# addtt/ladder-vae-pytorch

Measured on AMD Instinct MI355X. Metric: training images/sec (ELBO step: fwd+bwd+Adamax), higher is better.
Workload: dtype f32; 1 GPU; CIFAR10-shaped 15-layer LVAE (BASELINE configs[2]): 32x32x3, zdims 32x15, 4 blocks/layer, 64 filters, gated+skip, DMoL-10, dropout 0.2, free bits 1.0; batch_per_gpu=256, global_batch=256, parallelism=dp1, hip_graph=True

## Files before the change

### ladder-vae-pytorch_amd/csrc/conv3x3_bf16.hip

```cpp
#include <string.h>

#include "bf16_frag.h"
#include "bn_stats.h"
#include "lvae_host.h"

namespace lvae {

struct BfArgs {
  lvae_conv_desc d;
  const __bf16* Wp;
  int TH, TW, NI, tiles_h, halo_w, halo_h, halo_px, ntn, flip, Cin;
  uint32_t m_thw, m_tw, m_per_img, m_halo_w, m_tiles_h;
  int bm;
  int debug;
};

constexpr int BF_LDK = 72;

template <int SPLIT, int MI, bool PRE = false, bool XB = false, bool YB = false>
__global__ __launch_bounds__(256, 2) void conv3x3_bf16_kernel(BfArgs a) {
  kernarg_warmup<(sizeof(BfArgs) < 1024 ? sizeof(BfArgs) : 1024)>();
  static_assert(SPLIT == 1 || (!XB && !YB), "bf16 storage exists for the bf16-operand form only");
  constexpr int BM = 64 * MI, LDK = BF_LDK;
  extern __shared__ __attribute__((aligned(16))) unsigned char smem_raw[];
// ... 701 lines not shown
#pragma unroll
    for (int r = 0; r < 16; ++r) acc[j][r] = 0.f;
  f32x4 bsum = zero4, bsum8 = zero4;

  auto stage = [&](BfHRegs<XB, DB>& R, __bf16* Xs) {
    if (dbg & 2) return;
    __bf16* Ds = Xs + a.halo_px * LDK;
#pragma unroll
    for (int u = 0; u < (XB ? 2 : 4); ++u) {
      const int px = xpx + (XB ? 128 : 64) * u;
      if (px < a.halo_px) {
        if (XB) {
          bf16x8 w = R.x8[XB ? u : 0];
          if (d.in_scale && !(dbg & 16)) {
            f32x4 lo = {(float)w[0], (float)w[1], (float)w[2], (float)w[3]}, hi = {(float)w[4], (float)w[5], (float)w[6], (float)w[7]};
            lo = act_fwd4(lo * sc0 + sh0, d.in_act);
            hi = act_fwd4(hi * sc1 + sh1, d.in_act);
            w = to_bf16x8(lo, hi);
          }
          if (!((R.xok >> u) & 1u)) w = zero8;
          *reinterpret_cast<bf16x8*>(Xs + px * LDK + xcl) = w;
        } else {
          f32x4 w = zero4;
          if ((R.xok >> u) & 1u) {
            w = R.x4[XB ? 0 : u];
            if (d.in_scale && !(dbg & 16)) w = act_fwd4(w * sc0 + sh0, d.in_act);
          }
          *reinterpret_cast<bf16x4*>(Xs + px * LDK + xcl) = to_bf16x4(w);
        }
      }
    }
#pragma unroll
    for (int u = 0; u < (DB ? 2 : 4); ++u) {
      const int p = dpx + (DB ? 64 : 32) * u;
      if (DB) {
        const bf16x8 w = ((R.dok >> u) & 1u) ? R.d8[DB ? u : 0] : zero8;
        bsum += f32x4{(float)w[0], (float)w[1], (float)w[2], (float)w[3]};
        bsum8 += f32x4{(float)w[4], (float)w[5], (float)w[6], (float)w[7]};
        *reinterpret_cast<bf16x8*>(Ds + p * LDK + dcl) = w;
      } else {
        const f32x4 w = ((R.dok >> u) & 1u) ? R.d4[DB ? 0 : u] : zero4;
        bsum += w;
        *reinterpret_cast<bf16x4*>(Ds + p * LDK + dcl) = to_bf16x4(w);
      }
    }
  };
  auto mma_tile = [&](const __bf16* Xs) {
    if (dbg & 1) return;
    const __bf16* Ds = Xs + a.halo_px * LDK;
    const __bf16* Dl = Ds + drow0 * LDK + chd;
    int tb[3];
#pragma unroll
    for (int j = 0; j < 3; ++j) {
      tb[j] = tapoff[j];
      asm volatile("" : "+s"(tb[j]));
    }
#pragma unroll
    for (int s = 0; s < KS; ++s) {
      const bf16x8 bfr = tr_frag(Dl + 16 * s * LDK, Dl + (16 * s + 4) * LDK);
#pragma unroll
      for (int j = 0; j < 3; ++j) {
        if (j < ntap) {
          const bf16x8 afr = tr_frag(Xs + xoff[s][0] + tb[j], Xs + xoff[s][1] + tb[j]);
          acc[j] = __builtin_amdgcn_mfma_f32_32x32x16_bf16(afr, bfr, acc[j], 0, 0, 0);
        }
      }
      if (s & 1) __builtin_amdgcn_sched_barrier(0);
    }
  };

  BfHRegs<XB, DB> R0, R1;
  const int stride = nrange;
  int tile = range;
  if (tile < a.ntiles) prefetch(tile, R0);
  if (tile + stride < a.ntiles) prefetch(tile + stride, R1);
  for (; tile < a.ntiles; tile += 2 * stride) {
    stage(R0, buf0);
    __syncthreads();
    if (tile + 2 * stride < a.ntiles) prefetch(tile + 2 * stride, R0);
    mma_tile(buf0);
    if (tile + stride >= a.ntiles) break;
    stage(R1, buf0 + img_elems);
    __syncthreads();
    if (tile + 3 * stride < a.ntiles) prefetch(tile + 3 * stride, R1);
    mma_tile(buf0 + img_elems);
  }

  float* sw = a.slab_w + (size_t)range * 9 * Cin * d.Cout;
#pragma unroll
  for (int j = 0; j < 3; ++j) {
    if (j < ntap) {
      const int tap = tap0 + j;
#pragma unroll
      for (int r = 0; r < 16; ++r) {
        const int ci = cih * 32 + (r & 3) + 8 * (r >> 2) + 4 * lh, co = coh * 32 + li;
        if (!(dbg & 8) || acc[j][r] == 12345.678f) sw[((size_t)tap * Cin + ci) * d.Cout + co] = acc[j][r];
      }
    }
  }
  if (a.slab_b && cih == 0) {
    __syncthreads();
    float* red = reinterpret_cast<float*>(smem_raw);
    constexpr int NG = DB ? 64 : 32;
    if (DB) {
      *reinterpret_cast<f32x4*>(red + dpx * 64 + dcl) = bsum;
      *reinterpret_cast<f32x4*>(red + dpx * 64 + dcl + 4) = bsum8;
    } else {
      *reinterpret_cast<f32x4*>(red + dpx * 64 + dcl) = bsum;
    }
    __syncthreads();
    if (t < 64) {
      float v = 0.f;
#pragma unroll
      for (int g = 0; g < NG; ++g) v += red[g * 64 + t];
      a.slab_b[(size_t)range * d.Cout + t] = v;
    }
  }
}


__device__ __forceinline__ void bf_prep_element(const BfPrepEntry& e, int idx) {
  const int k = idx & 63, n = idx >> 6;
  if (n >= e.Npad) return;
  const int ntn = e.Npad >> 6, tn = n >> 6, nn = n & 63;
  for (int tap = 0; tap < 9; ++tap) {
    float r = (n < e.N && k < e.K) ? e.w[tap * e.stap + (int64_t)k * e.sk + (int64_t)n * e.sn] : 0.f;
    __bf16* dst = e.U + ((size_t)((tap * ntn + tn) * 4 + (k >> 4)) * e.kind * 2 + (nn >> 5)) * 512 + (((k >> 3) & 1) * 32 + (nn & 31)) * 8 + (k & 7);
    for (int p = 0; p < e.kind; ++p) {
      const __bf16 b = (__bf16)r;
      dst[(size_t)p * 1024] = b;
      r -= (float)b;
    }
  }
}

__device__ __forceinline__ void gate_prep_element(const BfPrepEntry& e, int idx) {
  const int planes = e.kind & 31;
  const int k = idx % e.K, n = idx / e.K;
  if (n >= e.N) return;
  float r = e.w[(int64_t)k * e.sk + (int64_t)n * e.sn];
  __bf16* dst = e.U + ((size_t)((k >> 4) * (e.N >> 5) + (n >> 5)) * planes) * 512 + (((k >> 3) & 1) * 32 + (n & 31)) * 8 + (k & 7);
  for (int p = 0; p < planes; ++p) {
    const __bf16 b = (__bf16)r;
    dst[(size_t)p * 512] = b;
    r -= (float)b;
  }
}

__global__ __launch_bounds__(256) void bf_weight_kernel(BfPrepEntry e) {
  if (e.kind & 32) gate_prep_element(e, blockIdx.x * 256 + threadIdx.x);
  else bf_prep_element(e, blockIdx.x * 256 + threadIdx.x);
}

__global__ __launch_bounds__(256) void bf_weight_batched_kernel(const BfPrepEntry* __restrict__ entries) {
  const BfPrepEntry e = entries[blockIdx.y];
  if (e.kind == 33 || e.kind == 35) {
    gate_prep_element(e, blockIdx.x * 256 + threadIdx.x);
    return;
  }
  if (e.kind != 1 && e.kind != 3) return;
  bf_prep_element(e, blockIdx.x * 256 + threadIdx.x);
}

int conv3x3_bf16_prepare_batched(const void* entries, int n, int npad, hipStream_t s) {
  hipLaunchKernelGGL(bf_weight_batched_kernel, dim3((npad * 64 + 255) / 256, n), dim3(256), 0, s, static_cast<const BfPrepEntry*>(entries));
  LVAE_LAUNCH_CHECK("bf_weight_batched");
  return 0;
}

size_t conv3x3_bf16_workspace(const lvae_conv_desc* d, int split) {
  const int ntn = (d->Cout + 63) / 64;
  return (size_t)9 * ntn * split * 4096 * sizeof(__bf16);
}

void conv3x3_bf16_prep_entry(const lvae_conv_desc* d, int split, void* entry) {
  BfPrepEntry e;
  e.w = d->w;
  e.U = static_cast<__bf16*>(d->workspace);
  e.stap = d->w_stap;
  e.sk = d->w_sk;
  e.sn = d->w_sn;
  e.K = d->C1;
  e.N = d->Cout;
  e.Npad = (d->Cout + 63) / 64 * 64;
  e.flip = 0;
  e.Kpad = 64;
  e.kind = split;
  memcpy(entry, &e, sizeof(e));
}

size_t resblock_gate_ws_bytes(const lvae_conv_desc* d, int planes) { return (size_t)d->C1 * d->Cout * planes * sizeof(__bf16); }
void resblock_gate_prep_entry(const lvae_conv_desc* d, int planes, void* entry) {
  BfPrepEntry e;
  e.w = d->w;
  e.U = static_cast<__bf16*>(d->workspace);
  e.stap = 0;
  e.sk = d->w_sk;
  e.sn = d->w_sn;
  e.K = d->C1;
  e.N = d->Cout;
  e.Npad = d->Cout;
  e.flip = 0;
  e.Kpad = d->C1;
  e.kind = 32 + planes;
  memcpy(entry, &e, sizeof(e));
}
int resblock_gate_prepare_single(const lvae_conv_desc* d, int planes, hipStream_t s) {
  BfPrepEntry e;
  resblock_gate_prep_entry(d, planes, &e);
  hipLaunchKernelGGL(bf_weight_kernel, dim3((e.K * e.N + 255) / 256), dim3(256), 0, s, e);
  LVAE_LAUNCH_CHECK("gate_weight");
  return 0;
}

int conv3x3_bf16_prepare_single(const lvae_conv_desc* d, int split, hipStream_t s) {
  BfPrepEntry e;
  conv3x3_bf16_prep_entry(d, split, &e);
  hipLaunchKernelGGL(bf_weight_kernel, dim3((e.Npad * 64 + 255) / 256), dim3(256), 0, s, e);
  LVAE_LAUNCH_CHECK("bf_weight");
  return 0;
}

static size_t bf_lds_bytes(int split, int halo_px, int bm) {
  const size_t in = (size_t)split * halo_px * BF_LDK * 2;
  const size_t out = (size_t)bm * 68 * 4;
  return in > out ? in : out;
}

static bool bf_plan_bm(const lvae_conv_desc* d, int split, int BM, BfArgs& a) {
  const int N = d->N, H = d->H, W = d->W;
  if (W > BM) return false;
  int TH = 1;
  for (int c = 1; c <= H; ++c)
    if (H % c == 0 && c * W <= BM) TH = c;
  int NI = BM / (TH * W);
  if (NI < 1) NI = 1;
  if (TH < H) NI = 1;
  if (NI > N) NI = N;
  a.TH = TH;
  a.TW = W;
  a.NI = NI;
  a.tiles_h = H / TH;
  a.halo_h = TH + 2;
  a.halo_w = W + 2;
  a.halo_px = NI * a.halo_h * a.halo_w;
  a.m_thw = fastdiv_magic(TH * W);
  a.m_tw = fastdiv_magic(W);
  a.m_per_img = fastdiv_magic(a.halo_h * a.halo_w);
  a.m_halo_w = fastdiv_magic(a.halo_w);
  a.bm = BM;
  return bf_lds_bytes(split, a.halo_px, BM) <= 160 * 1024;
}

static bool bf_plan(const lvae_conv_desc* d, int split, BfArgs& a) {
  if (bf_plan_bm(d, split, 128, a) && bf_lds_bytes(split, a.halo_px, 128) <= 80 * 1024 &&
      (int64_t)((d->N + a.NI - 1) / a.NI) * a.tiles_h * ((d->Cout + 63) / 64) >= 256)
    return true;
  if (bf_plan_bm(d, split, 64, a)) return true;
  return bf_plan_bm(d, split, 128, a);
}

static bool bf_select(const lvae_conv_desc* d, int split, BfArgs& a) {
  const int Cin = d->C1;
  if (d->KH != 3 || d->KW != 3 || d->stride != 1 || d->pad != 1 || d->x2 != nullptr || d->OH != d->H || d->OW != d->W) return false;
  if (d->in_fold != nullptr) return false;
  if (Cin > 64 || Cin % 4 != 0 || d->Cout % 4 != 0) return false;
  if ((int64_t)d->N * d->H * d->W * Cin >= ((int64_t)1 << 31)) return false;
  if (!al16_or_null(d->x) || !al16_or_null(d->y) || !al16_or_null(d->bias) || !al16_or_null(d->out_scale) || !al16_or_null(d->in_scale) || !al16_or_null(d->in_shift) ||
      !al16_or_null(d->stats_pivot) || !al16_or_null(d->stats_x))
    return false;
  a.d = *d;
  a.Cin = Cin;
  a.flip = d->gather == LVAE_GATHER_TRANSPOSED ? 1 : 0;
  return bf_plan(d, split, a);
}

static bool conv3x3_bf16_eligible(const lvae_conv_desc* d, int split) {
  BfArgs a;
  return bf_select(d, split, a);
}

int conv3x3_bf16_form(const lvae_conv_desc* d) {
  if (d->precision == LVAE_PREC_BF16) return conv3x3_bf16_eligible(d, 1) ? 1 : 0;
  const bool split_on = d->form == LVAE_FORM_SIX_PRODUCT_DIRECT;
  static const int64_t min_m = tune("LVAE_F32_SPLIT_MIN_M", 256 * 64);
  if (!split_on || (int64_t)d->N * d->H * d->W < min_m) return 0;
  return conv3x3_bf16_eligible(d, 3) ? 3 : 0;
}

bool conv3x3_bf16_plan(const lvae_conv_desc* d, bool assume_ws, ConvPlan& p) {
  const int split = conv3x3_bf16_form(d);
  if (split == 0) return false;
  const size_t ws = conv3x3_bf16_workspace(d, split);
  if (!assume_ws && (d->workspace == nullptr || (size_t)d->workspace_bytes < ws || !al16_or_null(d->workspace))) return false;
  BfArgs a;
  bf_select(d, split, a);
  p = ConvPlan{};
  p.variant = split == 1 ? LVAE_VARIANT_BF16_DIRECT : LVAE_VARIANT_SIX_DIRECT;
  p.rows = ((d->N + a.NI - 1) / a.NI) * a.tiles_h;
  p.workspace = ws;
  return true;
}

template <int SPLIT, int MI, bool PRE = false, bool XB = false, bool YB = false>
static int launch_bf(BfArgs a, hipStream_t s) {
  const int img_groups = (a.d.N + a.NI - 1) / a.NI;
  a.ntn = (a.d.Cout + 63) / 64;
  a.d.in_fold = nullptr;
  return launch_lds<conv3x3_bf16_kernel<SPLIT, MI, PRE, XB, YB>>("conv3x3_bf16", dim3(img_groups * a.tiles_h * a.ntn), dim3(256), bf_lds_bytes(SPLIT, a.halo_px, 64 * MI), 160 * 1024, s, a);
}

int conv3x3_bf16_launch(const lvae_conv_desc* d, const ConvPlan& p, hipStream_t s) {
  const int split = p.variant == LVAE_VARIANT_BF16_DIRECT ? 1 : 3;
  BfArgs a;
  bf_select(d, split, a);
  if (!d->workspace_ready) {
    BfPrepEntry e;
    conv3x3_bf16_prep_entry(d, split, &e);
// ... 126 lines not shown
```

### ladder-vae-pytorch_amd/csrc/conv3x3_wino.hip

```cpp
#include <stdlib.h>
#include <string.h>

#include "bf16_frag.h"
#include "bn_stats.h"
#include "lvae_host.h"

#ifndef LVAE_W1_RING
#define LVAE_W1_RING 3
#endif

namespace lvae {

struct WinoArgs {
  lvae_conv_desc d;
  const float* U;
  int TH, TW, NI, tiles_h, halo_w, halo_h, halo_px, ntn, Npad, tiles_x, wt_per_img, n_wt, Cin;
  uint32_t m_thw, m_per_img, m_halo_w, m_tiles_x, m_wt_per_img, m_tw;
  lvae_bn_fold f;
  int store_pivot;
  const __bf16* g_ws;
  const float* g_bias;
  const float* g_res;
  float* g_ab;
  float* g_out;
  float* g_stats;
  const float* g_pivot;
  int g_act;
};

__device__ __forceinline__ void store_u_split(__bf16* U3, int NB, int p, int k, int n, float v) {
  const size_t base = (((size_t)(p * 4 + (k >> 4)) * NB + (n >> 5)) * 3 * 64 + ((k >> 3) & 1) * 32 + (n & 31)) * 8 + (k & 7);
  float r = v;
#pragma unroll
  for (int q = 0; q < 3; ++q) {
    const __bf16 b = (__bf16)r;
    U3[base + (size_t)q * 512] = b;
    r -= (float)b;
  }
}

__global__ __launch_bounds__(256) void wino_weight_kernel(const float* __restrict__ w, int64_t stap, int64_t sk, int64_t sn,
                                                           int K, int Kpad, int N, int Npad, int flip, float* __restrict__ U, int split) {
  const int idx = blockIdx.x * 256 + threadIdx.x;
  if (idx >= Npad * Kpad) return;
  const int e = idx & 3, n = (idx >> 2) % Npad, kq = (idx >> 2) / Npad;
  const int k = kq * 4 + e;
  float g[3][3];
#pragma unroll
  for (int a = 0; a < 3; ++a)
#pragma unroll
    for (int b = 0; b < 3; ++b) {
      const int tap = flip ? (2 - a) * 3 + (2 - b) : a * 3 + b;
      g[a][b] = (n < N && k < K) ? w[tap * stap + (int64_t)k * sk + (int64_t)n * sn] : 0.f;
    }
  float t[4][3];
#pragma unroll
  for (int b = 0; b < 3; ++b) {
    t[0][b] = g[0][b];
    t[1][b] = 0.5f * (g[0][b] + g[1][b] + g[2][b]);
    t[2][b] = 0.5f * (g[0][b] - g[1][b] + g[2][b]);
    t[3][b] = g[2][b];
  }
  const size_t slab = (size_t)Npad * Kpad;
#pragma unroll
  for (int a = 0; a < 4; ++a) {
    const float u0 = t[a][0], u1 = 0.5f * (t[a][0] + t[a][1] + t[a][2]), u2 = 0.5f * (t[a][0] - t[a][1] + t[a][2]), u3 = t[a][2];
    if (split) {
      __bf16* U3 = reinterpret_cast<__bf16*>(U);
      store_u_split(U3, Npad >> 5, a * 4, k, n, u0);
      store_u_split(U3, Npad >> 5, a * 4 + 1, k, n, u1);
      store_u_split(U3, Npad >> 5, a * 4 + 2, k, n, u2);
      store_u_split(U3, Npad >> 5, a * 4 + 3, k, n, u3);
    } else {
      float* dst = U + (size_t)(a * 4) * slab + idx;
      dst[0] = u0;
      dst[slab] = u1;
      dst[2 * slab] = u2;
      dst[3 * slab] = u3;
    }
  }
}

struct WinoPrepEntry {
  const float* w;
  float* U;
  int64_t stap, sk, sn;
  int32_t K, N, Npad, flip;
  int32_t Kpad, pad_;
};
static_assert(sizeof(WinoPrepEntry) == 64, "entry layout is part of the C ABI (lvae_conv2d_prepare_entry)");

__global__ __launch_bounds__(256) void wino_weight_batched_kernel(const WinoPrepEntry* __restrict__ entries) {
  const WinoPrepEntry e = entries[blockIdx.y];
  const int idx = blockIdx.x * 256 + threadIdx.x;
  if (e.pad_ != 0 && e.pad_ != 16) return;
  if (idx >= e.Npad * e.Kpad) return;
  const int c = idx & 3, n = (idx >> 2) % e.Npad, kq = (idx >> 2) / e.Npad;
  const int k = kq * 4 + c;
  float g[3][3];
#pragma unroll
  for (int a = 0; a < 3; ++a)
#pragma unroll
    for (int b = 0; b < 3; ++b) {
      const int tap = e.flip ? (2 - a) * 3 + (2 - b) : a * 3 + b;
      g[a][b] = (n < e.N && k < e.K) ? e.w[tap * e.stap + (int64_t)k * e.sk + (int64_t)n * e.sn] : 0.f;
    }
  float t[4][3];
#pragma unroll
  for (int b = 0; b < 3; ++b) {
    t[0][b] = g[0][b];
    t[1][b] = 0.5f * (g[0][b] + g[1][b] + g[2][b]);
    t[2][b] = 0.5f * (g[0][b] - g[1][b] + g[2][b]);
    t[3][b] = g[2][b];
  }
  const size_t slab = (size_t)e.Npad * e.Kpad;
#pragma unroll
  for (int a = 0; a < 4; ++a) {
    const float u0 = t[a][0], u1 = 0.5f * (t[a][0] + t[a][1] + t[a][2]), u2 = 0.5f * (t[a][0] - t[a][1] + t[a][2]), u3 = t[a][2];
    if (e.pad_ == 16) {
      __bf16* U3 = reinterpret_cast<__bf16*>(e.U);
      store_u_split(U3, e.Npad >> 5, a * 4, k, n, u0);
      store_u_split(U3, e.Npad >> 5, a * 4 + 1, k, n, u1);
      store_u_split(U3, e.Npad >> 5, a * 4 + 2, k, n, u2);
      store_u_split(U3, e.Npad >> 5, a * 4 + 3, k, n, u3);
    } else {
      float* dst = e.U + (size_t)(a * 4) * slab + idx;
      dst[0] = u0;
      dst[slab] = u1;
      dst[2 * slab] = u2;
      dst[3 * slab] = u3;
    }
  }
}

constexpr int WLDO = 68;

template <int NT>
__device__ __forceinline__ void wino_fold_bn(const lvae_bn_fold& f, int C, float* scratch, float* coef, int t, bool writer) {
  constexpr int G = NT / 32;
  const int q = t & 31, g = t >> 5, rows = f.rows;
  f32x4 s = {0.f, 0.f, 0.f, 0.f};
  if (2 * q < C)
    for (int r = g; r < rows; r += 8 * G) {
      f32x4 p[8];
#pragma unroll
      for (int u = 0; u < 8; ++u) {
        const int rr = r + u * G;
        p[u] = *reinterpret_cast<const f32x4*>(f.parts + ((size_t)(rr < rows ? rr : 0) * 2) * C + 4 * q);
      }
#pragma unroll
      for (int u = 0; u < 8; ++u)
        if (r + u * G < rows) s += p[u];
    }
  *reinterpret_cast<f32x4*>(scratch + g * 128 + 4 * q) = s;
  __syncthreads();
  if (t < C) {
    double sa = 0.0, sb = 0.0;
#pragma unroll
    for (int k = 0; k < G; ++k) {
      sa += (double)scratch[k * 128 + t];
      sb += (double)scratch[k * 128 + C + t];
    }
    const float pivot = f.parts[((size_t)rows * 2) * C + t];
    const float gam = f.gamma ? f.gamma[t] : 1.f, bet = f.beta ? f.beta[t] : 0.f;
    const BnChannel r = bn_finalize_channel(sa, sb, pivot, f.M, f.eps, gam, bet);
    coef[t] = r.scale;
    coef[64 + t] = r.shift;
    if (writer) {
      if (f.coef_out) bn_store_coef(f.coef_out, C, t, r);
      if (f.running_mean) bn_update_running(f.running_mean, f.running_var, t, f.running_mean[t], f.running_var[t], f.momentum, r, f.M);
    }
  }
  __syncthreads();
}

#if defined(LVAE_WINO_DBG) && (LVAE_WINO_DBG & 64)
__device__ unsigned long long g_wino_stamps[8192 * 8];
#define WINO_STAMP(i)                                                                                           \
  do {                                                                                                          \
    if ((threadIdx.x & 63) == 0 && blockIdx.x < 1024)                                                           \
      g_wino_stamps[(blockIdx.x * (blockDim.x >> 6) + (threadIdx.x >> 6)) * 8 + (i)] = __builtin_amdgcn_s_memtime(); \
  } while (0)
#else
#define WINO_STAMP(i) do {} while (0)
#endif

template <int CIN, int NH, int MT, bool SPL>
__global__ __launch_bounds__(256, MT == 1 ? 2 : 1) void conv3x3_wino_kernel(WinoArgs a) {
  kernarg_warmup<(sizeof(WinoArgs) < 1024 ? sizeof(WinoArgs) : 1024)>();
  static_assert(!SPL || (CIN == 64 && MT == 1 && NH == 2), "six-product form: 64 reduction channels, 128-pixel workgroups");
  constexpr int WLDA = CIN + 4;
  constexpr int KSTEPS = CIN / 8, NSLICE = CIN / 16;
  constexpr int CW = 32 * NH;
  constexpr int C4N = CW / 4;
  constexpr int PG = 256 / C4N;
  constexpr int NT = 32 * MT;
  constexpr int QN = 4 * NT / PG;
  constexpr int RING = NH == 1 ? 3 : 2;
  extern __shared__ __attribute__((aligned(16))) float smem[];
  float* As = smem;
  const lvae_conv_desc& d = a.d;
  const int t = threadIdx.x, lane = t & 63, wave = t >> 6;
  const int li = lane & 31, lh = lane >> 5;
#ifdef LVAE_WINO_DBG
  constexpr int dbg = LVAE_WINO_DBG;
#else
  constexpr int dbg = 0;
#endif
  WINO_STAMP(0);
  int bid = blockIdx.x;
  {
    const int nwg = gridDim.x, xcd = bid & 7, q = nwg >> 3, r = nwg & 7;
    bid = (xcd < r ? xcd * (q + 1) : r * (q + 1) + (xcd - r) * q) + (bid >> 3);
  }
  const int tile_n = bid % a.ntn;
  const int tm = bid / a.ntn;
  const int th_idx = tm % a.tiles_h, ig = tm / a.tiles_h;
  const int n0 = ig * a.NI, oh0 = th_idx * a.TH, co0 = tile_n * CW;
  const f32x4 zero4 = {0.f, 0.f, 0.f, 0.f};

  constexpr int SLOTS = MT == 1 ? 4 : 6;
  const int per_img = a.halo_h * a.halo_w;
  const int hc4 = (t & 3) * 4;
  unsigned hoff[SLOTS];
  int hlds[SLOTS];
#pragma unroll
  for (int u = 0; u < SLOTS; ++u) {
    const int px = (t >> 2) + 64 * u;
    const int img = fastdiv(px, a.m_per_img), r = px - img * per_img;
    const int hy = fastdiv(r, a.m_halo_w), hx = r - hy * a.halo_w;
    const int n = n0 + img, ih = oh0 + hy - 1, iw = hx - 1;
    const bool ok = (n < d.N) & ((unsigned)ih < (unsigned)d.H) & ((unsigned)iw < (unsigned)d.W);
    hoff[u] = ok ? (unsigned)(((n * d.H + ih) * d.W + iw) * a.Cin + hc4) : ~0u;
    hlds[u] = px < a.halo_px ? px * WLDA + hc4 : -1;
  }
  f32x4 hreg[SLOTS];
  unsigned hlive = 0;
  auto load_slice = [&](int c) {
#pragma unroll
    for (int u = 0; u < SLOTS; ++u) {
      const bool live = hoff[u] != ~0u && 16 * c + hc4 < a.Cin;
      const unsigned off = live ? hoff[u] + 16 * c : 0u;
      if (dbg & 1) hreg[u] = zero4;
      else hreg[u] = *reinterpret_cast<const f32x4*>(d.x + off);
      hlive = live ? hlive | (1u << u) : hlive & ~(1u << u);
    }
  };
  __shared__ __attribute__((aligned(16))) float s_coef[128];
// ... 877 lines not shown
```

### ladder-vae-pytorch_amd/csrc/likelihood.hip

```cpp
#include "lvae_common.h"

namespace lvae {

__global__ __launch_bounds__(256) void bernoulli_fwd_kernel(const float* __restrict__ logits, const float* __restrict__ x,
                                                             const float* __restrict__ u, int64_t P, float* mean,
                                                             float* mode, float* sample, float* ll, float* dll) {
  __shared__ float red[4];
  const int n = blockIdx.x;
  const size_t base = (size_t)n * P;
  float acc = 0.f;
  for (int64_t i = threadIdx.x; i < P; i += 256) {
    const float lg = logits[base + i];
    const float m = sigmoidf_(lg);
    if (mean) mean[base + i] = m;
    if (mode) mode[base + i] = rintf(m);
    if (sample) sample[base + i] = u[base + i] < m ? 1.f : 0.f;
    if (x) {
      const float xv = x[base + i];
      const float l1 = fmaxf(lg < -20.f ? lg : logf(m), -100.f), l0 = fmaxf(logf(1.f - m), -100.f);
      acc += xv * l1 + (1.f - xv) * l0;
      if (dll) {
        const float v = m * (1.f - m);
        dll[base + i] = -(m - xv) / fmaxf(v, 1e-12f) * v;
      }
    }
  }
  if (x) {
    acc = block_sum_256(acc, red);
    if (threadIdx.x == 0) ll[n] = acc;
  }
}


struct ColourTerm {
  float lp, dmean, dls;
};

__device__ __forceinline__ ColourTerm dmol_colour(float x, float mean, float ls_raw) {
  ColourTerm r;
  const float ls = fmaxf(ls_raw, -7.f);
  const float inv_s = expf(-ls);
  const float cen = x - mean;
  const float plus = inv_s * (cen + 1.f / 255.f), mn = inv_s * (cen - 1.f / 255.f), mid = inv_s * cen;
  float dplus = 0.f, dmin = 0.f, dmid = 0.f, dls_direct = 0.f;
  if (x < -0.999f) {
    r.lp = plus - softplusf_(plus);
    dplus = 1.f - sigmoidf_(plus);
  } else if (x > 0.999f) {
    r.lp = -softplusf_(mn);
    dmin = -sigmoidf_(mn);
  } else {
    const float sp = sigmoidf_(plus), sm = sigmoidf_(mn);
    const float cdf_delta = sp - sm;
    if (cdf_delta > 1e-5f) {
      r.lp = logf(fmaxf(cdf_delta, 1e-12f));
      dplus = sp * (1.f - sp) / cdf_delta;
      dmin = -sm * (1.f - sm) / cdf_delta;
    } else {
      r.lp = mid - ls - 2.f * softplusf_(mid) - 4.8481163645876185f;
      dmid = 1.f - 2.f * sigmoidf_(mid);
      dls_direct = -1.f;
    }
  }
  r.dmean = -inv_s * (dplus + dmin + dmid);
  r.dls = (ls_raw >= -7.f) ? (-(plus * dplus + mn * dmin + mid * dmid) + dls_direct) : 0.f;
  return r;
}

template <int NMIX, int DM_PIX>
__global__ __launch_bounds__(DM_PIX) void dmol_ll_kernel(const float* __restrict__ l, const float* __restrict__ x,
                                                          int64_t npix, float* __restrict__ ll_pix,
                                                          float* __restrict__ dl) {
  constexpr int NP = 10 * NMIX, NPS = NP + 1;
  __shared__ float buf[DM_PIX * NPS];
  const int t = threadIdx.x;
  const int64_t p0 = (int64_t)blockIdx.x * DM_PIX;
  const int cnt = (int)min((int64_t)DM_PIX, npix - p0);
  const float* src = l + p0 * NP;
  for (int i = t; i < cnt * NP; i += DM_PIX) buf[(i / NP) * NPS + (i % NP)] = src[i];
  __syncthreads();
  if (t < cnt) {
    float* row = buf + t * NPS;
    const int64_t pix = p0 + t;
    const float x0 = 2.f * x[pix * 3 + 0] - 1.f, x1 = 2.f * x[pix * 3 + 1] - 1.f, x2 = 2.f * x[pix * 3 + 2] - 1.f;
    float lpk[NMIX];
    float lmax = -INFINITY;
#pragma unroll
    for (int k = 0; k < NMIX; ++k) lmax = fmaxf(lmax, row[k]);
    float lse = 0.f;
#pragma unroll
    for (int k = 0; k < NMIX; ++k) lse += expf(row[k] - lmax);
    lse = lmax + logf(lse);
    float best = -INFINITY;
#pragma unroll
    for (int k = 0; k < NMIX; ++k) {
      const float c0 = tanhf(row[NMIX + 2 * NMIX + k]);
      const float c1 = tanhf(row[NMIX + 3 * NMIX + 2 * NMIX + k]);
      const float c2 = tanhf(row[NMIX + 6 * NMIX + 2 * NMIX + k]);
      const float m0 = row[NMIX + k];
      const float m1 = row[NMIX + 3 * NMIX + k] + c0 * x0;
      const float m2 = row[NMIX + 6 * NMIX + k] + c1 * x0 + c2 * x1;
      const ColourTerm t0 = dmol_colour(x0, m0, row[NMIX + NMIX + k]);
      const ColourTerm t1 = dmol_colour(x1, m1, row[NMIX + 3 * NMIX + NMIX + k]);
      const ColourTerm t2 = dmol_colour(x2, m2, row[NMIX + 6 * NMIX + NMIX + k]);
      lpk[k] = t0.lp + t1.lp + t2.lp + (row[k] - lse);
      best = fmaxf(best, lpk[k]);
    }
    float se = 0.f;
#pragma unroll
    for (int k = 0; k < NMIX; ++k) se += expf(lpk[k] - best);
    const float llp = best + logf(se);
    ll_pix[pix] = llp;
    if (dl) {
#pragma unroll
      for (int k = 0; k < NMIX; ++k) {
        const float w = expf(lpk[k] - llp);
        const float logit = row[k];
        const float c0 = tanhf(row[NMIX + 2 * NMIX + k]);
        const float c1 = tanhf(row[NMIX + 3 * NMIX + 2 * NMIX + k]);
        const float c2 = tanhf(row[NMIX + 6 * NMIX + 2 * NMIX + k]);
        const float m0 = row[NMIX + k];
        const float m1 = row[NMIX + 3 * NMIX + k] + c0 * x0;
        const float m2 = row[NMIX + 6 * NMIX + k] + c1 * x0 + c2 * x1;
        const ColourTerm t0 = dmol_colour(x0, m0, row[NMIX + NMIX + k]);
        const ColourTerm t1 = dmol_colour(x1, m1, row[NMIX + 3 * NMIX + NMIX + k]);
        const ColourTerm t2 = dmol_colour(x2, m2, row[NMIX + 6 * NMIX + NMIX + k]);
        row[k] = w - expf(logit - lse);
        row[NMIX + k] = w * t0.dmean;
        row[NMIX + NMIX + k] = w * t0.dls;
        row[NMIX + 2 * NMIX + k] = w * t1.dmean * x0 * (1.f - c0 * c0);
        row[NMIX + 3 * NMIX + k] = w * t1.dmean;
        row[NMIX + 3 * NMIX + NMIX + k] = w * t1.dls;
        row[NMIX + 3 * NMIX + 2 * NMIX + k] = w * t2.dmean * x0 * (1.f - c1 * c1);
        row[NMIX + 6 * NMIX + k] = w * t2.dmean;
        row[NMIX + 6 * NMIX + NMIX + k] = w * t2.dls;
        row[NMIX + 6 * NMIX + 2 * NMIX + k] = w * t2.dmean * x1 * (1.f - c2 * c2);
      }
    }
  }
  if (dl) {
    __syncthreads();
    float* dst = dl + p0 * NP;
    for (int i = t; i < cnt * NP; i += DM_PIX) dst[i] = buf[(i / NP) * NPS + (i % NP)];
  }
}

__global__ __launch_bounds__(256) void rowsum_kernel(const float* __restrict__ v, int64_t P, float* out) {
  __shared__ float red[4];
  const int n = blockIdx.x;
  float acc = 0.f;
  for (int64_t i = threadIdx.x; i < P; i += 256) acc += v[(size_t)n * P + i];
  acc = block_sum_256(acc, red);
  if (threadIdx.x == 0) out[n] = acc;
}

template <int NMIX>
__global__ __launch_bounds__(256) void dmol_sample_kernel(const float* __restrict__ l, const float* __restrict__ u_mix,
                                                           const float* __restrict__ u_log, int64_t npix,
                                                           float* __restrict__ sample) {
  constexpr int NP = 10 * NMIX;
  for (int64_t pix = (int64_t)blockIdx.x * 256 + threadIdx.x; pix < npix; pix += (int64_t)gridDim.x * 256) {
    const float* row = l + pix * NP;
    int sel = 0;
    float best = -INFINITY;
#pragma unroll
    for (int k = 0; k < NMIX; ++k) {
      const float g = row[k] - logf(-logf(u_mix[pix * NMIX + k]));
      if (g > best) {
        best = g;
        sel = k;
      }
    }
    float xs[3], co[3];
#pragma unroll
    for (int c = 0; c < 3; ++c) {
      const float mean = row[NMIX + 3 * NMIX * c + sel];
      const float ls = fmaxf(row[NMIX + 3 * NMIX * c + NMIX + sel], -7.f);
      co[c] = tanhf(row[NMIX + 3 * NMIX * c + 2 * NMIX + sel]);
      const float u = u_log[pix * 3 + c];
      xs[c] = mean + expf(ls) * (logf(u) - logf(1.f - u));
    }
    const float x0 = fminf(fmaxf(xs[0], -1.f), 1.f);
    const float x1 = fminf(fmaxf(xs[1] + co[0] * x0, -1.f), 1.f);
    const float x2 = fminf(fmaxf(xs[2] + co[1] * x0 + co[2] * x1, -1.f), 1.f);
    sample[pix * 3 + 0] = fminf(fmaxf((x0 + 1.f) * 0.5f, 0.f), 1.f);
    sample[pix * 3 + 1] = fminf(fmaxf((x1 + 1.f) * 0.5f, 0.f), 1.f);
    sample[pix * 3 + 2] = fminf(fmaxf((x2 + 1.f) * 0.5f, 0.f), 1.f);
  }
}

__global__ __launch_bounds__(256) void gaussian_fwd_kernel(const float* __restrict__ params, const float* __restrict__ x,
                                                            const float* __restrict__ eps, int64_t P, int C, float* sample,
                                                            float* ll, float* dll) {
  __shared__ float red[4];
  const int n = blockIdx.x;
  const int64_t per = P * C;
  float acc = 0.f;
  for (int64_t i = threadIdx.x; i < per; i += 256) {
    const int64_t pix = i / C;
    const int c = (int)(i - pix * C);
    const size_t pb = ((size_t)n * P + pix) * 2 * C;
    const float mean = params[pb + c], lv = params[pb + C + c];
    if (sample) sample[(size_t)n * per + i] = mean + expf(0.5f * lv) * eps[(size_t)n * per + i];
    if (x) {
      const float d = x[(size_t)n * per + i] - mean, iv = expf(-lv);
      acc += -0.5f * (d * d * iv + lv + 1.8378770664093453f);
      if (dll) {
        dll[pb + c] = d * iv;
        dll[pb + C + c] = -0.5f * (1.f - d * d * iv);
      }
    }
  }
  if (x) {
    acc = block_sum_256(acc, red);
    if (threadIdx.x == 0) ll[n] = acc;
  }
}

__global__ __launch_bounds__(256) void discr_logistic_fwd_kernel(const float* __restrict__ raw, const float* __restrict__ x,
                                                                  const float* __restrict__ u, int64_t P, int C,
                                                                  float* mean_out, float* ls_out, float* sample, float* ll,
                                                                  float* dll) {
  __shared__ float red[4];
  const int n = blockIdx.x;
  const int64_t per = P * C;
  const float nb = 256.f;
  float acc = 0.f;
  for (int64_t i = threadIdx.x; i < per; i += 256) {
    const int64_t pix = i / C;
    const int c = (int)(i - pix * C);
    const size_t pb = ((size_t)n * P + pix) * 2 * C, oi = (size_t)n * per + i;
    const float mean = raw[pb + c] + 0.5f;
    const float ls_raw = raw[pb + C + c] - 1.f;
    const float ls = fmaxf(ls_raw, -7.f);
    const float scale = expf(ls);
    if (mean_out) mean_out[oi] = mean;
    if (ls_out) ls_out[oi] = ls;
    if (sample) {
      const float uu = u[oi];
      sample[oi] = fminf(fmaxf(mean + scale * (logf(uu) - logf(1.f - uu)), 0.f), 1.f);
    }
    if (x) {
      const float xs = x[oi] * (255.f / 256.f) + 1.f / 512.f;
      const float xq = floorf(xs * nb) / nb;
      const bool has_plus = xq < (nb - 1.f) / nb, has_minus = xq >= 1.f / nb;
      const float a = (xq + 1.f / nb - mean) / scale, b = (xq - mean) / scale;
      const float sa = sigmoidf_(a), sb = sigmoidf_(b);
      const float cp = has_plus ? sa : 1.f, cm = has_minus ? sb : 0.f;
      const float prob = cp - cm + 1e-7f;
      acc += logf(prob);
      if (dll) {
        const float da = has_plus ? sa * (1.f - sa) : 0.f, db = has_minus ? sb * (1.f - sb) : 0.f;
        dll[pb + c] = -(da - db) / scale / prob;
        dll[pb + C + c] = (ls_raw >= -7.f) ? -(a * da - b * db) / prob : 0.f;
      }
    }
  }
  if (x) {
    acc = block_sum_256(acc, red);
    if (threadIdx.x == 0) ll[n] = acc;
  }
}

__global__ __launch_bounds__(256) void scale_per_sample_kernel(const float* __restrict__ a, const float* __restrict__ g,
                                                                int64_t P, int64_t total, float* __restrict__ out) {
  for (int64_t i = (int64_t)blockIdx.x * 256 + threadIdx.x; i < total; i += (int64_t)gridDim.x * 256)
    out[i] = a[i] * g[i / P];
}

}

using namespace lvae;

extern "C" int lvae_bernoulli_fwd_f32(const float* logits, const float* x, const float* u, int32_t N, int64_t P,
                                      float* mean, float* mode, float* sample, float* ll, float* dll_dlogits,
                                      void* stream) {
  LVAE_REQUIRE(logits && N > 0 && P > 0, LVAE_EINVAL, "lvae_bernoulli_fwd_f32: bad args");
  LVAE_REQUIRE(!sample || u, LVAE_EINVAL, "lvae_bernoulli_fwd_f32: sample needs uniforms");
  LVAE_REQUIRE(!x || ll, LVAE_EINVAL, "lvae_bernoulli_fwd_f32: x given but ll is null");
  hipLaunchKernelGGL(bernoulli_fwd_kernel, dim3(N), dim3(256), 0, (hipStream_t)stream, logits, x, u, P, mean, mode, sample,
                     ll, dll_dlogits);
  LVAE_LAUNCH_CHECK("bernoulli_fwd");
  return 0;
}

extern "C" size_t lvae_dmol_workspace(int32_t N, int32_t HW) { return (size_t)N * HW * sizeof(float); }

#define LVAE_DMOL_COUNTS(X) X(1) X(2) X(3) X(4) X(5) X(6) X(8) X(10) X(12) X(16) X(20)
static bool dmol_supported(int nmix) {
  switch (nmix) {
#define X(n) case n:
    LVAE_DMOL_COUNTS(X)
#undef X
    return true;
    default: return false;
  }
}

extern "C" int lvae_dmol_ll_fwd_f32(const float* l, const float* x, int32_t N, int32_t HW, int32_t nmix, float* ll,
                                    float* dll_dl, void* workspace, size_t workspace_bytes, void* stream) {
  LVAE_REQUIRE(l && x && ll && workspace && N > 0 && HW > 0, LVAE_EINVAL, "lvae_dmol_ll_fwd_f32: bad args");
  LVAE_REQUIRE(dmol_supported(nmix), LVAE_EINVAL, "lvae_dmol_ll_fwd_f32: %d mixture components: instantiated for 1-6, 8, 10, 12, 16, 20", nmix);
  LVAE_REQUIRE(workspace_bytes >= lvae_dmol_workspace(N, HW), LVAE_EWORKSPACE, "lvae_dmol_ll_fwd_f32: workspace");
  const int64_t npix = (int64_t)N * HW;
  hipStream_t s = (hipStream_t)stream;
  float* ll_pix = static_cast<float*>(workspace);
  switch (nmix) {
#define X(n)                                                                                                                         \
  case n: {                                                                                                                          \
    constexpr int PIX = (128 * (10 * n + 1) * 4 <= 64 * 1024) ? 128 : 64;                                                            \
    hipLaunchKernelGGL((dmol_ll_kernel<n, PIX>), dim3((unsigned)((npix + PIX - 1) / PIX)), dim3(PIX), 0, s, l, x, npix, ll_pix, dll_dl); \
  } break;
    LVAE_DMOL_COUNTS(X)
#undef X
  }
  LVAE_LAUNCH_CHECK("dmol_ll");
  hipLaunchKernelGGL(rowsum_kernel, dim3(N), dim3(256), 0, s, ll_pix, (int64_t)HW, ll);
  LVAE_LAUNCH_CHECK("dmol_rowsum");
  return 0;
}

extern "C" int lvae_dmol_sample_f32(const float* l, const float* u_mix, const float* u_log, int32_t N, int32_t HW,
                                    int32_t nmix, float* sample, void* stream) {
  LVAE_REQUIRE(l && u_mix && u_log && sample && N > 0 && HW > 0, LVAE_EINVAL, "lvae_dmol_sample_f32: bad args");
  LVAE_REQUIRE(dmol_supported(nmix), LVAE_EINVAL, "lvae_dmol_sample_f32: %d mixture components: instantiated for 1-6, 8, 10, 12, 16, 20", nmix);
  const int64_t npix = (int64_t)N * HW;
  switch (nmix) {
#define X(n) \
  case n: hipLaunchKernelGGL(dmol_sample_kernel<n>, dim3(grid_for(npix, 256)), dim3(256), 0, (hipStream_t)stream, l, u_mix, u_log, npix, sample); break;
    LVAE_DMOL_COUNTS(X)
#undef X
  }
  LVAE_LAUNCH_CHECK("dmol_sample");
  return 0;
}

extern "C" int lvae_scale_per_sample_f32(const float* a, const float* g, int32_t N, int64_t P, float* out, void* stream) {
  LVAE_REQUIRE(a && g && out && N > 0 && P > 0, LVAE_EINVAL, "lvae_scale_per_sample_f32: bad args");
  const int64_t total = (int64_t)N * P;
  hipLaunchKernelGGL(scale_per_sample_kernel, dim3(grid_for(total, 256)), dim3(256), 0, (hipStream_t)stream, a, g, P,
                     total, out);
  LVAE_LAUNCH_CHECK("scale_per_sample");
  return 0;
}

extern "C" int lvae_gaussian_fwd_f32(const float* params, const float* x, const float* eps, int32_t N, int64_t P, int32_t C,
                                     float* sample, float* ll, float* dll_dparams, void* stream) {
  LVAE_REQUIRE(params && N > 0 && P > 0 && C > 0, LVAE_EINVAL, "lvae_gaussian_fwd_f32: bad args");
  LVAE_REQUIRE(!sample || eps, LVAE_EINVAL, "lvae_gaussian_fwd_f32: sample needs eps");
  LVAE_REQUIRE(!x || ll, LVAE_EINVAL, "lvae_gaussian_fwd_f32: x given but ll is null");
  hipLaunchKernelGGL(gaussian_fwd_kernel, dim3(N), dim3(256), 0, (hipStream_t)stream, params, x, eps, P, C, sample, ll,
                     dll_dparams);
  LVAE_LAUNCH_CHECK("gaussian_fwd");
  return 0;
}

extern "C" int lvae_discr_logistic_fwd_f32(const float* raw, const float* x, const float* u, int32_t N, int64_t P, int32_t C,
                                           float* mean, float* logscale, float* sample, float* ll, float* dll_draw,
                                           void* stream) {
  LVAE_REQUIRE(raw && N > 0 && P > 0 && C > 0, LVAE_EINVAL, "lvae_discr_logistic_fwd_f32: bad args");
  LVAE_REQUIRE(!sample || u, LVAE_EINVAL, "lvae_discr_logistic_fwd_f32: sample needs uniforms");
  LVAE_REQUIRE(!x || ll, LVAE_EINVAL, "lvae_discr_logistic_fwd_f32: x given but ll is null");
  hipLaunchKernelGGL(discr_logistic_fwd_kernel, dim3(N), dim3(256), 0, (hipStream_t)stream, raw, x, u, P, C, mean, logscale,
                     sample, ll, dll_draw);
  LVAE_LAUNCH_CHECK("discr_logistic_fwd");
  return 0;
}
```

Before: 8897 images/s.

## Parallelize DMoL likelihood across mixtures and tile weight-prep kernels through LDS

The DMoL log-likelihood kernel now gives each mixture component its own lane, using wave shuffles for the log-sum-exp reductions, and drops the duplicated forward recompute in the gradient pass. Staging to and from shared memory uses unpadded, 16-byte vectorized copies. The bf16 and Winograd weight-prep kernels are restructured into per-tile LDS transposes with vectorized bf16x8 split-plane stores in place of scattered per-element writes. This brings more parallelism and more coalesced memory traffic, at the cost of added code paths, LDS bank conflicts on the unpadded buffer, and lanes wasted when the mixture count is not a power of two (10 mixtures leaves 6 of 16 lanes idle).

```diff
diff --git a/ladder-vae-pytorch_amd/csrc/conv3x3_bf16.hip b/ladder-vae-pytorch_amd/csrc/conv3x3_bf16.hip
--- a/ladder-vae-pytorch_amd/csrc/conv3x3_bf16.hip
+++ b/ladder-vae-pytorch_amd/csrc/conv3x3_bf16.hip
@@ -877,18 +877,125 @@
   else bf_prep_element(e, blockIdx.x * 256 + threadIdx.x);
 }
 
+template <int SPLIT>
+__device__ __forceinline__ void store_split8(__bf16* dst, size_t plane_stride, float (&r)[8]) {
+#pragma unroll
+  for (int p = 0; p < SPLIT; ++p) {
+    bf16x8 v;
+#pragma unroll
+    for (int j = 0; j < 8; ++j) {
+      const __bf16 b = (__bf16)r[j];
+      v[j] = b;
+      r[j] -= (float)b;
+    }
+    *reinterpret_cast<bf16x8*>(dst + (size_t)p * plane_stride) = v;
+  }
+}
+
+constexpr int BWLD = 65;
+template <int SPLIT>
+__device__ __forceinline__ void bf_prep_block(const BfPrepEntry& e, int block, float* tile) {
+  const int tap = block % 9, tn = block / 9, ntn = e.Npad >> 6;
+  if (tn >= ntn) return;
+  const int t = threadIdx.x, n0 = tn * 64;
+  const float* w = e.w + tap * e.stap;
+  const bool al = ((reinterpret_cast<uintptr_t>(e.w) & 15) | (e.stap & 3)) == 0;
+  if (al && e.sn == 1 && (e.sk & 3) == 0) {
+#pragma unroll
+    for (int i = 0; i < 4; ++i) {
+      const int k = (t >> 4) + 16 * i, c = (t & 15) * 4, n = n0 + c;
+      const float* src = w + (int64_t)k * e.sk + n;
+      f32x4 v = {0.f, 0.f, 0.f, 0.f};
+      if (k < e.K) {
+        if (n + 3 < e.N) {
+          v = *reinterpret_cast<const f32x4*>(src);
+        } else {
+#pragma unroll
+          for (int j = 0; j < 4; ++j)
+            if (n + j < e.N) v[j] = src[j];
+        }
+      }
+#pragma unroll
+      for (int j = 0; j < 4; ++j) tile[k * BWLD + c + j] = v[j];
+    }
+  } else if (al && e.sk == 1 && (e.sn & 3) == 0) {
+#pragma unroll
+    for (int i = 0; i < 4; ++i) {
+      const int nn = (t >> 4) + 16 * i, k = (t & 15) * 4, n = n0 + nn;
+      const float* src = w + (int64_t)n * e.sn + k;
+      f32x4 v = {0.f, 0.f, 0.f, 0.f};
+      if (n < e.N) {
+        if (k + 3 < e.K) {
+          v = *reinterpret_cast<const f32x4*>(src);
+        } else {
+#pragma unroll
+          for (int j = 0; j < 4; ++j)
+            if (k + j < e.K) v[j] = src[j];
+        }
+      }
+#pragma unroll
+      for (int j = 0; j < 4; ++j) tile[(k + j) * BWLD + nn] = v[j];
+    }
+  } else {
+#pragma unroll 4
+    for (int i = 0; i < 16; ++i) {
+      const int k = t & 63, nn = (t >> 6) + 4 * i, n = n0 + nn;
+      tile[k * BWLD + nn] = (n < e.N && k < e.K) ? w[(int64_t)k * e.sk + (int64_t)n * e.sn] : 0.f;
+    }
+  }
+  __syncthreads();
+#pragma unroll
+  for (int i = 0; i < 2; ++i) {
+    const int c = t + 256 * i, lane = c & 63, nh = (c >> 6) & 1, ks = c >> 7;
+    const int k0 = ks * 16 + (lane >> 5) * 8, nn = nh * 32 + (lane & 31);
+    float r[8];
+#pragma unroll
+    for (int j = 0; j < 8; ++j) r[j] = tile[(k0 + j) * BWLD + nn];
+    store_split8<SPLIT>(e.U + ((size_t)((tap * ntn + tn) * 4 + ks) * SPLIT * 2 + nh) * 512 + lane * 8, 1024, r);
+  }
+}
+
+template <int SPLIT>
+__device__ __forceinline__ void gate_prep_block(const BfPrepEntry& e, int first, int stride) {
+  const bool kvec = e.sk == 1 && (e.sn & 3) == 0 && (reinterpret_cast<uintptr_t>(e.w) & 15) == 0;
+  const int ntile = e.N >> 5, groups = (e.K >> 4) * ntile * 64;
+  for (int g = first; g < groups; g += stride) {
+    const int lane = g & 63, nt = (g >> 6) % ntile, ks = (g >> 6) / ntile;
+    const int k0 = ks * 16 + (lane >> 5) * 8, n = nt * 32 + (lane & 31);
+    const float* src = e.w + (int64_t)k0 * e.sk + (int64_t)n * e.sn;
+    float r[8];
+    if (kvec) {
+      const f32x4 a = *reinterpret_cast<const f32x4*>(src), b = *reinterpret_cast<const f32x4*>(src + 4);
+#pragma unroll
+      for (int j = 0; j < 4; ++j) r[j] = a[j], r[4 + j] = b[j];
+    } else {
+#pragma unroll
+      for (int j = 0; j < 8; ++j) r[j] = src[(int64_t)j * e.sk];
+    }
+    store_split8<SPLIT>(e.U + ((size_t)(ks * ntile + nt) * SPLIT) * 512 + lane * 8, 512, r);
+  }
+}
+
 __global__ __launch_bounds__(256) void bf_weight_batched_kernel(const BfPrepEntry* __restrict__ entries) {
+  __shared__ float tile[64 * BWLD];
   const BfPrepEntry e = entries[blockIdx.y];
   if (e.kind == 33 || e.kind == 35) {
-    gate_prep_element(e, blockIdx.x * 256 + threadIdx.x);
+    const int first = blockIdx.x * 256 + threadIdx.x, stride = gridDim.x * 256;
+    if ((e.K & 15) || (e.N & 31)) {
+      for (int idx = first; idx < e.K * e.N; idx += stride) gate_prep_element(e, idx);
+    } else if (e.kind == 33) {
+      gate_prep_block<1>(e, first, stride);
+    } else {
+      gate_prep_block<3>(e, first, stride);
+    }
     return;
   }
-  if (e.kind != 1 && e.kind != 3) return;
-  bf_prep_element(e, blockIdx.x * 256 + threadIdx.x);
+  if (e.kind == 1) bf_prep_block<1>(e, blockIdx.x, tile);
+  else if (e.kind == 3) bf_prep_block<3>(e, blockIdx.x, tile);
 }
 
 int conv3x3_bf16_prepare_batched(const void* entries, int n, int npad, hipStream_t s) {
-  hipLaunchKernelGGL(bf_weight_batched_kernel, dim3((npad * 64 + 255) / 256, n), dim3(256), 0, s, static_cast<const BfPrepEntry*>(entries));
+  hipLaunchKernelGGL(bf_weight_batched_kernel, dim3(9 * (npad / 64), n), dim3(256), 0, s, static_cast<const BfPrepEntry*>(entries));
   LVAE_LAUNCH_CHECK("bf_weight_batched");
   return 0;
 }
diff --git a/ladder-vae-pytorch_amd/csrc/conv3x3_wino.hip b/ladder-vae-pytorch_amd/csrc/conv3x3_wino.hip
--- a/ladder-vae-pytorch_amd/csrc/conv3x3_wino.hip
+++ b/ladder-vae-pytorch_amd/csrc/conv3x3_wino.hip
@@ -90,10 +90,74 @@
 };
 static_assert(sizeof(WinoPrepEntry) == 64, "entry layout is part of the C ABI (lvae_conv2d_prepare_entry)");
 
+constexpr int WPLD = 33;
+__device__ __forceinline__ void wino_prep_split_tile(const WinoPrepEntry& e, int tile, float* u) {
+  const int NB = e.Npad >> 5;
+  if (tile >= (e.Kpad >> 4) * NB) return;
+  const int ks = tile / NB, nb = tile % NB, t = threadIdx.x;
+#pragma unroll
+  for (int i = 0; i < 2; ++i) {
+    const int it = t + 256 * i;
+    const int kk = e.sk == 1 ? (it & 15) : (it >> 5), nl = e.sk == 1 ? (it >> 4) : (it & 31);
+    const int k = ks * 16 + kk, n = nb * 32 + nl;
+    float g[3][3];
+#pragma unroll
+    for (int a = 0; a < 3; ++a)
+#pragma unroll
+      for (int b = 0; b < 3; ++b) {
+        const int tap = e.flip ? (2 - a) * 3 + (2 - b) : a * 3 + b;
+        g[a][b] = (n < e.N && k < e.K) ? e.w[tap * e.stap + (int64_t)k * e.sk + (int64_t)n * e.sn] : 0.f;
+      }
+    float tt[4][3];
+#pragma unroll
+    for (int b = 0; b < 3; ++b) {
+      tt[0][b] = g[0][b];
+      tt[1][b] = 0.5f * (g[0][b] + g[1][b] + g[2][b]);
+      tt[2][b] = 0.5f * (g[0][b] - g[1][b] + g[2][b]);
+      tt[3][b] = g[2][b];
+    }
+    float* dst = u + kk * WPLD + nl;
+#pragma unroll
+    for (int a = 0; a < 4; ++a) {
+      dst[(a * 4 + 0) * 16 * WPLD] = tt[a][0];
+      dst[(a * 4 + 1) * 16 * WPLD] = 0.5f * (tt[a][0] + tt[a][1] + tt[a][2]);
+      dst[(a * 4 + 2) * 16 * WPLD] = 0.5f * (tt[a][0] - tt[a][1] + tt[a][2]);
+      dst[(a * 4 + 3) * 16 * WPLD] = tt[a][2];
+    }
+  }
+  __syncthreads();
+  __bf16* U3 = reinterpret_cast<__bf16*>(e.U);
+#pragma unroll
+  for (int i = 0; i < 4; ++i) {
+    const int it = t + 256 * i, lane = it & 63, p = it >> 6;
+    const float* src = u + (p * 16 + (lane >> 5) * 8) * WPLD + (lane & 31);
+    float r[8];
+#pragma unroll
+    for (int j = 0; j < 8; ++j) r[j] = src[j * WPLD];
+    __bf16* dst = U3 + ((((size_t)(p * 4 + ks) * NB + nb) * 3 * 64) + lane) * 8;
+#pragma unroll
+    for (int q = 0; q < 3; ++q) {
+      bf16x8 v;
+#pragma unroll
+      for (int j = 0; j < 8; ++j) {
+        const __bf16 h = (__bf16)r[j];
+        v[j] = h;
+        r[j] -= (float)h;
+      }
+      *reinterpret_cast<bf16x8*>(dst + (size_t)q * 512) = v;
+    }
+  }
+}
+
 __global__ __launch_bounds__(256) void wino_weight_batched_kernel(const WinoPrepEntry* __restrict__ entries) {
+  __shared__ float u_lds[16 * 16 * WPLD];
   const WinoPrepEntry e = entries[blockIdx.y];
   const int idx = blockIdx.x * 256 + threadIdx.x;
   if (e.pad_ != 0 && e.pad_ != 16) return;
+  if (e.pad_ == 16 && e.Kpad == 64) {
+    wino_prep_split_tile(e, blockIdx.x, u_lds);
+    return;
+  }
   if (idx >= e.Npad * e.Kpad) return;
   const int c = idx & 3, n = (idx >> 2) % e.Npad, kq = (idx >> 2) / e.Npad;
   const int k = kq * 4 + c;
diff --git a/ladder-vae-pytorch_amd/csrc/likelihood.hip b/ladder-vae-pytorch_amd/csrc/likelihood.hip
--- a/ladder-vae-pytorch_amd/csrc/likelihood.hip
+++ b/ladder-vae-pytorch_amd/csrc/likelihood.hip
@@ -67,81 +67,87 @@
   return r;
 }
 
+constexpr int dmol_lanes(int nmix) { return nmix <= 1 ? 1 : nmix <= 2 ? 2 : nmix <= 4 ? 4 : nmix <= 8 ? 8 : nmix <= 16 ? 16 : 32; }
+
+template <int LPP>
+__device__ __forceinline__ float group_max(float v) {
+#pragma unroll
+  for (int m = 1; m < LPP; m <<= 1) v = fmaxf(v, __shfl_xor(v, m, 64));
+  return v;
+}
+template <int LPP>
+__device__ __forceinline__ float group_sum(float v) {
+#pragma unroll
+  for (int m = 1; m < LPP; m <<= 1) v += __shfl_xor(v, m, 64);
+  return v;
+}
+
 template <int NMIX, int DM_PIX>
-__global__ __launch_bounds__(DM_PIX) void dmol_ll_kernel(const float* __restrict__ l, const float* __restrict__ x,
-                                                          int64_t npix, float* __restrict__ ll_pix,
-                                                          float* __restrict__ dl) {
-  constexpr int NP = 10 * NMIX, NPS = NP + 1;
-  __shared__ float buf[DM_PIX * NPS];
+__global__ __launch_bounds__(DM_PIX * dmol_lanes(NMIX)) void dmol_ll_kernel(const float* __restrict__ l, const float* __restrict__ x,
+                                                                            int64_t npix, float* __restrict__ ll_pix,
+                                                                            float* __restrict__ dl) {
+  constexpr int NP = 10 * NMIX, LPP = dmol_lanes(NMIX), NT = DM_PIX * LPP;
+  static_assert((DM_PIX * NP) % 4 == 0, "a workgroup's block of rows starts 16-byte aligned");
+  __shared__ __attribute__((aligned(16))) float buf[DM_PIX * NP];
   const int t = threadIdx.x;
   const int64_t p0 = (int64_t)blockIdx.x * DM_PIX;
   const int cnt = (int)min((int64_t)DM_PIX, npix - p0);
+  const int nflt = cnt * NP, nvec = nflt >> 2;
   const float* src = l + p0 * NP;
-  for (int i = t; i < cnt * NP; i += DM_PIX) buf[(i / NP) * NPS + (i % NP)] = src[i];
+  const bool vec = ((reinterpret_cast<uintptr_t>(l) | reinterpret_cast<uintptr_t>(dl)) & 15) == 0;
+  if (vec) {
+    for (int i = t; i < nvec; i += NT) reinterpret_cast<f32x4*>(buf)[i] = reinterpret_cast<const f32x4*>(src)[i];
+    for (int i = nvec * 4 + t; i < nflt; i += NT) buf[i] = src[i];
+  } else {
+    for (int i = t; i < nflt; i += NT) buf[i] = src[i];
+  }
   __syncthreads();
-  if (t < cnt) {
-    float* row = buf + t * NPS;
-    const int64_t pix = p0 + t;
+  {
+    const int pl = t / LPP, kl = t % LPP;
+    const bool active = pl < cnt && kl < NMIX;
+    const int p = min(pl, cnt - 1), k = min(kl, NMIX - 1);
+    float* row = buf + p * NP;
+    const int64_t pix = p0 + p;
     const float x0 = 2.f * x[pix * 3 + 0] - 1.f, x1 = 2.f * x[pix * 3 + 1] - 1.f, x2 = 2.f * x[pix * 3 + 2] - 1.f;
-    float lpk[NMIX];
-    float lmax = -INFINITY;
-#pragma unroll
-    for (int k = 0; k < NMIX; ++k) lmax = fmaxf(lmax, row[k]);
-    float lse = 0.f;
-#pragma unroll
-    for (int k = 0; k < NMIX; ++k) lse += expf(row[k] - lmax);
-    lse = lmax + logf(lse);
-    float best = -INFINITY;
-#pragma unroll
-    for (int k = 0; k < NMIX; ++k) {
-      const float c0 = tanhf(row[NMIX + 2 * NMIX + k]);
-      const float c1 = tanhf(row[NMIX + 3 * NMIX + 2 * NMIX + k]);
-      const float c2 = tanhf(row[NMIX + 6 * NMIX + 2 * NMIX + k]);
-      const float m0 = row[NMIX + k];
-      const float m1 = row[NMIX + 3 * NMIX + k] + c0 * x0;
-      const float m2 = row[NMIX + 6 * NMIX + k] + c1 * x0 + c2 * x1;
-      const ColourTerm t0 = dmol_colour(x0, m0, row[NMIX + NMIX + k]);
-      const ColourTerm t1 = dmol_colour(x1, m1, row[NMIX + 3 * NMIX + NMIX + k]);
-      const ColourTerm t2 = dmol_colour(x2, m2, row[NMIX + 6 * NMIX + NMIX + k]);
-      lpk[k] = t0.lp + t1.lp + t2.lp + (row[k] - lse);
-      best = fmaxf(best, lpk[k]);
-    }
-    float se = 0.f;
-#pragma unroll
-    for (int k = 0; k < NMIX; ++k) se += expf(lpk[k] - best);
-    const float llp = best + logf(se);
-    ll_pix[pix] = llp;
-    if (dl) {
-#pragma unroll
-      for (int k = 0; k < NMIX; ++k) {
-        const float w = expf(lpk[k] - llp);
-        const float logit = row[k];
-        const float c0 = tanhf(row[NMIX + 2 * NMIX + k]);
-        const float c1 = tanhf(row[NMIX + 3 * NMIX + 2 * NMIX + k]);
-        const float c2 = tanhf(row[NMIX + 6 * NMIX + 2 * NMIX + k]);
-        const float m0 = row[NMIX + k];
-        const float m1 = row[NMIX + 3 * NMIX + k] + c0 * x0;
-        const float m2 = row[NMIX + 6 * NMIX + k] + c1 * x0 + c2 * x1;
-        const ColourTerm t0 = dmol_colour(x0, m0, row[NMIX + NMIX + k]);
-        const ColourTerm t1 = dmol_colour(x1, m1, row[NMIX + 3 * NMIX + NMIX + k]);
-        const ColourTerm t2 = dmol_colour(x2, m2, row[NMIX + 6 * NMIX + NMIX + k]);
-        row[k] = w - expf(logit - lse);
-        row[NMIX + k] = w * t0.dmean;
-        row[NMIX + NMIX + k] = w * t0.dls;
-        row[NMIX + 2 * NMIX + k] = w * t1.dmean * x0 * (1.f - c0 * c0);
-        row[NMIX + 3 * NMIX + k] = w * t1.dmean;
-        row[NMIX + 3 * NMIX + NMIX + k] = w * t1.dls;
-        row[NMIX + 3 * NMIX + 2 * NMIX + k] = w * t2.dmean * x0 * (1.f - c1 * c1);
-        row[NMIX + 6 * NMIX + k] = w * t2.dmean;
-        row[NMIX + 6 * NMIX + NMIX + k] = w * t2.dls;
-        row[NMIX + 6 * NMIX + 2 * NMIX + k] = w * t2.dmean * x1 * (1.f - c2 * c2);
-      }
+    const float logit = row[k];
+    const float lmax = group_max<LPP>(kl < NMIX ? logit : -INFINITY);
+    const float lse = lmax + logf(group_sum<LPP>(kl < NMIX ? expf(logit - lmax) : 0.f));
+    const float c0 = tanhf(row[NMIX + 2 * NMIX + k]);
+    const float c1 = tanhf(row[NMIX + 3 * NMIX + 2 * NMIX + k]);
+    const float c2 = tanhf(row[NMIX + 6 * NMIX + 2 * NMIX + k]);
+    const float m0 = row[NMIX + k];
+    const float m1 = row[NMIX + 3 * NMIX + k] + c0 * x0;
+    const float m2 = row[NMIX + 6 * NMIX + k] + c1 * x0 + c2 * x1;
+    const ColourTerm t0 = dmol_colour(x0, m0, row[NMIX + NMIX + k]);
+    const ColourTerm t1 = dmol_colour(x1, m1, row[NMIX + 3 * NMIX + NMIX + k]);
+    const ColourTerm t2 = dmol_colour(x2, m2, row[NMIX + 6 * NMIX + NMIX + k]);
+    const float lpk = t0.lp + t1.lp + t2.lp + (logit - lse);
+    const float best = group_max<LPP>(kl < NMIX ? lpk : -INFINITY);
+    const float llp = best + logf(group_sum<LPP>(kl < NMIX ? expf(lpk - best) : 0.f));
+    if (active && kl == 0) ll_pix[pix] = llp;
+    if (dl && active) {
+      const float w = expf(lpk - llp);
+      row[k] = w - expf(logit - lse);
+      row[NMIX + k] = w * t0.dmean;
+      row[NMIX + NMIX + k] = w * t0.dls;
+      row[NMIX + 2 * NMIX + k] = w * t1.dmean * x0 * (1.f - c0 * c0);
+      row[NMIX + 3 * NMIX + k] = w * t1.dmean;
+      row[NMIX + 3 * NMIX + NMIX + k] = w * t1.dls;
+      row[NMIX + 3 * NMIX + 2 * NMIX + k] = w * t2.dmean * x0 * (1.f - c1 * c1);
+      row[NMIX + 6 * NMIX + k] = w * t2.dmean;
+      row[NMIX + 6 * NMIX + NMIX + k] = w * t2.dls;
+      row[NMIX + 6 * NMIX + 2 * NMIX + k] = w * t2.dmean * x1 * (1.f - c2 * c2);
     }
   }
   if (dl) {
     __syncthreads();
     float* dst = dl + p0 * NP;
-    for (int i = t; i < cnt * NP; i += DM_PIX) dst[i] = buf[(i / NP) * NPS + (i % NP)];
+    if (vec) {
+      for (int i = t; i < nvec; i += NT) reinterpret_cast<f32x4*>(dst)[i] = reinterpret_cast<const f32x4*>(buf)[i];
+      for (int i = nvec * 4 + t; i < nflt; i += NT) dst[i] = buf[i];
+    } else {
+      for (int i = t; i < nflt; i += NT) dst[i] = buf[i];
+    }
   }
 }
 
@@ -308,8 +314,8 @@
   switch (nmix) {
 #define X(n)                                                                                                                         \
   case n: {                                                                                                                          \
-    constexpr int PIX = (128 * (10 * n + 1) * 4 <= 64 * 1024) ? 128 : 64;                                                            \
-    hipLaunchKernelGGL((dmol_ll_kernel<n, PIX>), dim3((unsigned)((npix + PIX - 1) / PIX)), dim3(PIX), 0, s, l, x, npix, ll_pix, dll_dl); \
+    constexpr int PIX = 256 / dmol_lanes(n);                                                      \
+    hipLaunchKernelGGL((dmol_ll_kernel<n, PIX>), dim3((unsigned)((npix + PIX - 1) / PIX)), dim3(256), 0, s, l, x, npix, ll_pix, dll_dl); \
   } break;
     LVAE_DMOL_COUNTS(X)
 #undef X
```

Result: no change. 8960 images/s, median of 6 (+0.7%).
